# lslrh/DynaMask

Measured on AMD Instinct MI355X. Metric: img/s (DynaMask mask-head path, 512 RoIs/img, fixed 28x28 exit; ms_per_step = ms per RoI batch), higher is better.
Workload: dtype f32

## Files before the change

dynamask_amd/csrc/deform_conv.hip:

```cpp
#include "common.h"

namespace {

struct DcnArgs {
  const float* x;
  const float* offset;
  int NB, C, H, W, HW, Q;
  const float* wp;
  int Cout, CoutP, KQ, dg, relu;
  int q_begin = 0;
  float* out;
  int MT;
  float* ws = nullptr;
  long long ws_stride = 0, ws_floats = 0;
  int ksplit = 1, kchan = 0;
  const float* w2t = nullptr;
  const float* b2 = nullptr;
  float* out2 = nullptr;
  int M2 = 0, w2_ld = 0, out2_ct = 0, store_out = 1;
};

__device__ __forceinline__ float dcn_bilinear(float wt0, float wt1, float wb0, float wb1, float ta, float tb, float ba, float bb) {
  return __builtin_fmaf(wb1, bb, __builtin_fmaf(wb0, ba, __builtin_fmaf(wt1, tb, wt0 * ta)));
}

template <int WGM, int WGN, int WM, int WN>
__global__ __launch_bounds__(WGM* WGN * 64) void deform_conv_kernel(DcnArgs a) {
  constexpr int CK = 8;
  constexpr int TM = WGM * WM * 32;
  constexpr int TN = WGN * WN * 32;
  constexpr int NT = WGM * WGN * 64;
  constexpr int TG = NT / TN;
  constexpr int MAXT = (9 + TG - 1) / TG;
  constexpr int A_F4 = 9 * 2 * TM;
  constexpr int A_PER_T = (A_F4 + NT - 1) / NT;
  static_assert(NT % TN == 0, "threads must tile the pixel columns");

  extern __shared__ __attribute__((aligned(16))) float lds[];
  const int kc_begin = (a.ksplit > 1) ? (int)blockIdx.y * a.kchan : 0;
  const int kc_end = (a.ksplit > 1) ? min(a.C, kc_begin + a.kchan) : a.C;
  float* const e_out = (a.ksplit > 1) ? a.ws + (size_t)blockIdx.y * a.ws_stride : a.out;
  const int e_relu = (a.ksplit > 1) ? 0 : a.relu;
  dm_f32x4* ldsA = reinterpret_cast<dm_f32x4*>(lds);
  dm_f32x4* ldsB = reinterpret_cast<dm_f32x4*>(lds) + A_F4;

  const int tid = threadIdx.x;
  const int lane = tid & 63, wave = tid >> 6;
  const int wave_m = wave / WGN, wave_n = wave % WGN;
  const int hi = lane >> 5, l31 = lane & 31;
  int m_tile, n_tile;
  {
    const int b = blockIdx.x, grp = 8 * a.MT;
    const int full = (gridDim.x / grp) * grp;
    if (b < full) {
      const int g = b / grp, r = b - g * grp;
      m_tile = r / 8;
      n_tile = g * 8 + (r & 7);
    } else {
      const int r = b - full;
      m_tile = r % a.MT;
      n_tile = full / a.MT + r / a.MT;
    }
  }
  const int m0 = m_tile * TM;
  const int q0 = a.q_begin + n_tile * TN;
  const int HW = a.HW, W = a.W, H = a.H;

  int col_n[WN], col_p[WN];
  bool col_ok[WN];
#pragma unroll
  for (int wn = 0; wn < WN; ++wn) {
    int q = q0 + (wave_n * WN + wn) * 32 + l31;
    col_ok[wn] = q < a.Q;
    q = min(q, a.Q - 1);
    col_n[wn] = q / HW;
    col_p[wn] = q - col_n[wn] * HW;
  }

  const int gj = tid % TN;
  const int tg = tid / TN;
  int gq = q0 + gj;
  const bool g_ok = gq < a.Q;
  gq = min(gq, a.Q - 1);
  const int gn = gq / HW;
  const int gp = gq - gn * HW;
  const int gy = gp / W, gx = gp - gy * W;

  int ot[MAXT], ob[MAXT];
  float wt0[MAXT], wt1[MAXT], wb0[MAXT], wb1[MAXT];
  int cur_group = -1;
  const int cpg = a.C / a.dg;

  auto load_params = [&](int group) {
    const float* offp = a.offset + ((size_t)gn * a.dg + group) * 18 * HW + gp;
#pragma unroll
    for (int t = 0; t < MAXT; ++t) {
      const int tap = tg + t * TG;
      ot[t] = ob[t] = 0;
      wt0[t] = wt1[t] = wb0[t] = wb1[t] = 0.f;
      if (tap < 9 && g_ok) {
        const int ki = tap / 3, kj = tap - ki * 3;
        const float off_h = offp[(size_t)(2 * tap) * HW];
        const float off_w = offp[(size_t)(2 * tap + 1) * HW];
        const float h_im = (float)(gy - 1 + ki) + off_h;
        const float w_im = (float)(gx - 1 + kj) + off_w;
        if (h_im > -1.f && w_im > -1.f && h_im < (float)H && w_im < (float)W) {
          const int h_low = (int)floorf(h_im), w_low = (int)floorf(w_im);
          const float lh = h_im - (float)h_low, lw = w_im - (float)w_low;
          const float hh = 1.f - lh, hw = 1.f - lw;
          const float wr_t = (h_low >= 0) ? hh : 0.f;
          const float wr_b = (h_low + 1 <= H - 1) ? lh : 0.f;
          const int rt = min(max(h_low, 0), H - 1), rbm = min(max(h_low + 1, 0), H - 1);
          const int cb = min(max(w_low, 0), W - 2);
          const float wc0 = (cb == w_low ? hw : 0.f) + (cb == w_low + 1 ? lw : 0.f);
          const float wc1 = (cb + 1 == w_low ? hw : 0.f) + (cb + 1 == w_low + 1 ? lw : 0.f);
          ot[t] = rt * W + cb;
          ob[t] = rbm * W + cb;
          wt0[t] = wr_t * wc0; wt1[t] = wr_t * wc1;
          wb0[t] = wr_b * wc0; wb1[t] = wr_b * wc1;
        }
      }
    }
  };

  dm_f32x16 acc[WM][WN];
#pragma unroll
  for (int i = 0; i < WM; ++i)
#pragma unroll
    for (int j = 0; j < WN; ++j)
#pragma unroll
      for (int r = 0; r < 16; ++r) acc[i][j][r] = 0.f;

  struct __attribute__((packed, aligned(4))) F2 { float a, b; };
  dm_f32x4 ra[A_PER_T];
  dm_f32x4 raw[MAXT * 4];
  dm_f32x4 rb0[MAXT];

  auto prefetch_a = [&](int c0) {
#pragma unroll
    for (int i = 0; i < A_PER_T; ++i) {
      const int idx = tid + i * NT;
      dm_f32x4 v = {0.f, 0.f, 0.f, 0.f};
      if (idx < A_F4) {
        const int m = idx % TM;
        const int tq = idx / TM;
        const int qd = tq & 1;
        const int tap = tq >> 1;
        if (m0 + m < a.CoutP)
          v = *reinterpret_cast<const dm_f32x4*>(a.wp + (((size_t)tap * a.KQ + (c0 >> 2) + qd) * a.CoutP + m0 + m) * 4);
      }
      ra[i] = v;
    }
  };
  auto issue_quad = [&](int c0, int qd) {
    const float* xp = a.x + ((size_t)gn * a.C + c0 + qd * 4) * HW;
#pragma unroll
    for (int t = 0; t < MAXT; ++t) {
#pragma unroll
      for (int e = 0; e < 4; ++e) {
        const float* xc = xp + (size_t)e * HW;
        const F2 top = *reinterpret_cast<const F2*>(xc + ot[t]);
        const F2 bot = *reinterpret_cast<const F2*>(xc + ob[t]);
        dm_f32x4 v = {top.a, top.b, bot.a, bot.b};
        raw[t * 4 + e] = v;
      }
    }
  };
  auto combine = [&](int t) {
    dm_f32x4 v;
#pragma unroll
    for (int e = 0; e < 4; ++e) {
      const dm_f32x4 l = raw[t * 4 + e];
      v[e] = dcn_bilinear(wt0[t], wt1[t], wb0[t], wb1[t], l[0], l[1], l[2], l[3]);
    }
    return v;
  };
  auto commit = [&]() {
#pragma unroll
    for (int i = 0; i < A_PER_T; ++i) {
      const int idx = tid + i * NT;
      if (idx < A_F4) ldsA[idx] = ra[i];
    }
#pragma unroll
    for (int t = 0; t < MAXT; ++t) {
      const int tap = tg + t * TG;
      if (tap < 9) {
        ldsB[(0 * 9 + tap) * TN + gj] = rb0[t];
        ldsB[(1 * 9 + tap) * TN + gj] = combine(t);
      }
    }
  };
  auto load_frag = [&](int tap, dm_f32x4* av, dm_f32x4* bv) {
#pragma unroll
    for (int i = 0; i < WM; ++i) av[i] = ldsA[(tap * 2 + hi) * TM + (wave_m * WM + i) * 32 + l31];
#pragma unroll
    for (int j = 0; j < WN; ++j) bv[j] = ldsB[(hi * 9 + tap) * TN + (wave_n * WN + j) * 32 + l31];
  };
  auto mfma_taps = [&](int t0, int t1) {
    dm_f32x4 av[2][WM], bv[2][WN];
    load_frag(t0, av[0], bv[0]);
#pragma unroll
    for (int tap = t0; tap < t1; ++tap) {
      const int cur = (tap - t0) & 1;
      if (tap + 1 < t1) load_frag(tap + 1, av[cur ^ 1], bv[cur ^ 1]);
#pragma unroll
      for (int e = 0; e < 4; ++e)
#pragma unroll
        for (int i = 0; i < WM; ++i)
#pragma unroll
          for (int j = 0; j < WN; ++j)
            acc[i][j] = __builtin_amdgcn_mfma_f32_32x32x2f32(av[cur][i][e], bv[cur][j][e], acc[i][j], 0, 0, 0);
    }
  };

  cur_group = kc_begin / cpg;
  load_params(cur_group);
  prefetch_a(kc_begin);
  issue_quad(kc_begin, 0);
#pragma unroll
  for (int t = 0; t < MAXT; ++t) rb0[t] = combine(t);
  issue_quad(kc_begin, 1);

  for (int c0 = kc_begin; c0 < kc_end; c0 += CK) {
    commit();
    __syncthreads();
    const int cn = c0 + CK;
    const bool more = cn < kc_end;
    if (more) {
      const int group = cn / cpg;
      if (group != cur_group) {
        cur_group = group;
        load_params(group);
      }
      prefetch_a(cn);
      issue_quad(cn, 0);
    }
    __builtin_amdgcn_sched_barrier(0);
    mfma_taps(0, 4);
    __builtin_amdgcn_sched_barrier(0);
    if (more) {
#pragma unroll
      for (int t = 0; t < MAXT; ++t) rb0[t] = combine(t);
      issue_quad(cn, 1);
    }
    __builtin_amdgcn_sched_barrier(0);
    mfma_taps(4, 9);
    __syncthreads();
  }

  {
    float* pj[WN];
#pragma unroll
    for (int j = 0; j < WN; ++j) pj[j] = e_out + (size_t)col_n[j] * a.Cout * HW + col_p[j];
    const int co_lane = m0 + wave_m * WM * 32 + 4 * hi;
    const size_t off_lane = (size_t)co_lane * HW;
    const bool relu = e_relu != 0;
#pragma unroll
    for (int i = 0; i < WM; ++i) {
#pragma unroll
      for (int r = 0; r < 16; ++r) {
        const int k = i * 32 + (r & 3) + 8 * (r >> 2);
        if (co_lane + k < a.Cout) {
          const size_t o = off_lane + (size_t)k * HW;
#pragma unroll
          for (int j = 0; j < WN; ++j) {
            if (col_ok[j]) {
              float v = acc[i][j][r];
              if (relu) v = fmaxf(v, 0.f);
              pj[j][o] = v;
            }
          }
        }
      }
    }
  }
}

__global__ __launch_bounds__(256, 2) void deform_conv_lds_kernel(DcnArgs a) {
  constexpr int TM = 128, TN = 128, NT = 256;
  constexpr int AS_F4 = 3 * 2 * TM;
  constexpr int BS_F4 = 3 * 2 * TN;
  constexpr int A_PER_T = AS_F4 / NT;
  constexpr int X_PER_T = 4;
  extern __shared__ __attribute__((aligned(16))) float lds[];
  const int kc_begin = (a.ksplit > 1) ? (int)blockIdx.y * a.kchan : 0;
  const int kc_end = (a.ksplit > 1) ? min(a.C, kc_begin + a.kchan) : a.C;
  float* const e_out = (a.ksplit > 1) ? a.ws + (size_t)blockIdx.y * a.ws_stride : a.out;
  const int e_relu = (a.ksplit > 1) ? 0 : a.relu;
  dm_f32x4* ldsA = reinterpret_cast<dm_f32x4*>(lds);
  dm_f32x4* ldsB = ldsA + 2 * AS_F4;
  dm_f32x4* ldsX = ldsB + 2 * BS_F4;

  const int tid = threadIdx.x, lane = tid & 63, wave = tid >> 6;
  const int wave_m = wave >> 1, wave_n = wave & 1;
  const int hi = lane >> 5, l31 = lane & 31;
  int m_tile, n_tile;
  {
    const int b = blockIdx.x, grp = 8 * a.MT;
    const int full = (gridDim.x / grp) * grp;
    if (b < full) {
      const int g = b / grp, r = b - g * grp;
      m_tile = r / 8;
      n_tile = g * 8 + (r & 7);
    } else {
      const int r = b - full;
      m_tile = r % a.MT;
      n_tile = full / a.MT + r / a.MT;
    }
  }
  const int m0 = m_tile * TM, q0 = a.q_begin + n_tile * TN;
  const int HW = a.HW, W = a.W, H = a.H;
  const int n0 = q0 / HW;
  const int xbuf = 2 * 2 * HW;

  int col_n[2], col_p[2];
  bool col_ok[2];
#pragma unroll
  for (int wn = 0; wn < 2; ++wn) {
    int q = q0 + (wave_n * 2 + wn) * 32 + l31;
    col_ok[wn] = q < a.Q;
    q = min(q, a.Q - 1);
    col_n[wn] = q / HW;
    col_p[wn] = q - col_n[wn] * HW;
  }

  const int gj = tid & 127, gh = tid >> 7;
  int gq = q0 + gj;
  const bool g_ok = gq < a.Q;
  gq = min(gq, a.Q - 1);
  const int gn = gq / HW, gp = gq - gn * HW;
  const int gy = gp / W, gx = gp - gy * W;
  const int xbase = ((gn - n0) * 2 + gh) * HW;

  int otb[9];
  float wt0[9], wt1[9], wb0[9], wb1[9];
  const int cpg = a.C / a.dg;
  auto load_params = [&](int group) {
    const float* offp = a.offset + ((size_t)gn * a.dg + group) * 18 * HW + gp;
#pragma unroll
    for (int tap = 0; tap < 9; ++tap) {
      otb[tap] = 0;
      wt0[tap] = wt1[tap] = wb0[tap] = wb1[tap] = 0.f;
      if (g_ok) {
        const int ki = tap / 3, kj = tap - ki * 3;
        const float h_im = (float)(gy - 1 + ki) + offp[(size_t)(2 * tap) * HW];
        const float w_im = (float)(gx - 1 + kj) + offp[(size_t)(2 * tap + 1) * HW];
        if (h_im > -1.f && w_im > -1.f && h_im < (float)H && w_im < (float)W) {
          const int h_low = (int)floorf(h_im), w_low = (int)floorf(w_im);
          const float lh = h_im - (float)h_low, lw = w_im - (float)w_low;
          const float hh = 1.f - lh, hw = 1.f - lw;
          const float wr_t = (h_low >= 0) ? hh : 0.f;
          const float wr_b = (h_low + 1 <= H - 1) ? lh : 0.f;
          const int rt = min(max(h_low, 0), H - 1), rbm = min(max(h_low + 1, 0), H - 1);
          const int cb = min(max(w_low, 0), W - 2);
          const float wc0 = (cb == w_low ? hw : 0.f) + (cb == w_low + 1 ? lw : 0.f);
          const float wc1 = (cb + 1 == w_low ? hw : 0.f) + (cb + 1 == w_low + 1 ? lw : 0.f);
          otb[tap] = (rt * W + cb) | ((rbm * W + cb) << 16);
          wt0[tap] = wr_t * wc0; wt1[tap] = wr_t * wc1;
          wb0[tap] = wr_b * wc0; wb1[tap] = wr_b * wc1;
        }
      }
    }
  };

  dm_f32x16 acc[2][2];
#pragma unroll
  for (int i = 0; i < 2; ++i)
#pragma unroll
    for (int j = 0; j < 2; ++j)
#pragma unroll
      for (int r = 0; r < 16; ++r) acc[i][j][r] = 0.f;

  dm_f32x4 ra[A_PER_T], rx[X_PER_T];
  int x_off[X_PER_T];
#pragma unroll
  for (int i = 0; i < X_PER_T; ++i) {
    const int idx = tid + i * NT;
    const int img = idx / (2 * HW), r = idx - img * 2 * HW;
    const int quad = r / HW, px = r - quad * HW;
    const int ii = (idx < 4 * HW) ? img : 0, qq = (idx < 4 * HW) ? quad : 0, pp = (idx < 4 * HW) ? px : 0;
    x_off[i] = ((min(n0 + ii, a.NB - 1) - n0) * a.C + qq * 4) * HW + pp;
  }
  auto load_a = [&](int c0, int g) {
#pragma unroll
    for (int i = 0; i < A_PER_T; ++i) {
      const int idx = tid + i * NT;
      const int m = idx % TM, tq = idx / TM;
      const int mm = min(m0 + m, a.CoutP - 1);
      ra[i] = *reinterpret_cast<const dm_f32x4*>(a.wp + (((size_t)(3 * g + (tq >> 1)) * a.KQ + (c0 >> 2) + (tq & 1)) * a.CoutP + mm) * 4);
    }
  };
  auto store_a = [&](int slot) {
#pragma unroll
    for (int i = 0; i < A_PER_T; ++i) ldsA[slot * AS_F4 + tid + i * NT] = ra[i];
  };
  auto load_x = [&](int c0) {
    const float* xc = a.x + ((size_t)n0 * a.C + c0) * HW;
#pragma unroll
    for (int i = 0; i < X_PER_T; ++i) {
#pragma unroll
      for (int e = 0; e < 4; ++e) rx[i][e] = xc[x_off[i] + e * HW];
    }
  };
  auto store_x = [&](int buf) {
#pragma unroll
    for (int i = 0; i < X_PER_T; ++i) {
      const int idx = tid + i * NT;
      if (idx < 4 * HW) ldsX[buf * xbuf + idx] = rx[i];
    }
  };
  auto gather3 = [&](int t0, int slot, int buf) {
    const dm_f32x4* xq = ldsX + buf * xbuf + xbase;
#pragma unroll
    for (int u = 0; u < 3; ++u) {
      const int tap = t0 + u;
      const dm_f32x4* pt = xq + (otb[tap] & 0xffff);
      const dm_f32x4* pb = xq + (otb[tap] >> 16);
      const dm_f32x4 tl = pt[0], tr = pt[1], bl = pb[0], br = pb[1];
      dm_f32x4 v;
#pragma unroll
      for (int e = 0; e < 4; ++e) v[e] = dcn_bilinear(wt0[tap], wt1[tap], wb0[tap], wb1[tap], tl[e], tr[e], bl[e], br[e]);
      ldsB[slot * BS_F4 + (u * 2 + gh) * TN + gj] = v;
    }
  };
  auto step = [&](int slot, bool fill, int t0, int gbuf) {
    const dm_f32x4* xq = ldsX + gbuf * xbuf + xbase;
#pragma unroll
    for (int u = 0; u < 3; ++u) {
      dm_f32x4 av[2], bv[2];
#pragma unroll
      for (int i = 0; i < 2; ++i) av[i] = ldsA[slot * AS_F4 + (u * 2 + hi) * TM + (wave_m * 2 + i) * 32 + l31];
#pragma unroll
      for (int j = 0; j < 2; ++j) bv[j] = ldsB[slot * BS_F4 + (u * 2 + hi) * TN + (wave_n * 2 + j) * 32 + l31];
      const int tap = t0 + u;
      dm_f32x4 tl, tr, bl, br;
      if (fill) {
        const dm_f32x4* pt = xq + (otb[tap] & 0xffff);
        const dm_f32x4* pb = xq + (otb[tap] >> 16);
        tl = pt[0]; tr = pt[1]; bl = pb[0]; br = pb[1];
      }
      __builtin_amdgcn_sched_barrier(0);
#pragma unroll
      for (int e = 0; e < 2; ++e)
#pragma unroll
        for (int i = 0; i < 2; ++i)
#pragma unroll
          for (int j = 0; j < 2; ++j) acc[i][j] = __builtin_amdgcn_mfma_f32_32x32x2f32(av[i][e], bv[j][e], acc[i][j], 0, 0, 0);
      __builtin_amdgcn_sched_barrier(0);
      if (fill) {
        dm_f32x4 v;
#pragma unroll
        for (int e = 0; e < 4; ++e) v[e] = dcn_bilinear(wt0[tap], wt1[tap], wb0[tap], wb1[tap], tl[e], tr[e], bl[e], br[e]);
        ldsB[(slot ^ 1) * BS_F4 + (u * 2 + gh) * TN + gj] = v;
      }
      __builtin_amdgcn_sched_barrier(0);
#pragma unroll
      for (int e = 2; e < 4; ++e)
#pragma unroll
        for (int i = 0; i < 2; ++i)
#pragma unroll
          for (int j = 0; j < 2; ++j) acc[i][j] = __builtin_amdgcn_mfma_f32_32x32x2f32(av[i][e], bv[j][e], acc[i][j], 0, 0, 0);
      __builtin_amdgcn_sched_barrier(0);
    }
  };

  int cur_group = kc_begin / cpg;
  load_params(cur_group);
  load_x(kc_begin);
  load_a(kc_begin, 0);
  store_x(0);
  store_a(0);
  load_a(kc_begin, 1);
  __syncthreads();
  gather3(0, 0, 0);
  __syncthreads();
  int slot = 0;
  for (int c0 = kc_begin, buf = 0; c0 < kc_end; c0 += 8, buf ^= 1) {
    const int cn = c0 + 8;
    const bool more = cn < kc_end;
    if (more) load_x(cn);
    store_a(slot ^ 1);
    load_a(c0, 2);
    step(slot, true, 3, buf);
    __syncthreads();
    slot ^= 1;
    store_a(slot ^ 1);
    if (more) {
      load_a(cn, 0);
      store_x(buf ^ 1);
    }
    step(slot, true, 6, buf);
    __syncthreads();
    slot ^= 1;
    if (more) {
      const int group = cn / cpg;
      if (group != cur_group) {
        cur_group = group;
        load_params(group);
      }
      store_a(slot ^ 1);
      load_a(cn, 1);
    }
    step(slot, more, 0, buf ^ 1);
    __syncthreads();
    slot ^= 1;
  }

  {
    float* pj[2];
#pragma unroll
    for (int j = 0; j < 2; ++j) pj[j] = e_out + (size_t)col_n[j] * a.Cout * HW + col_p[j];
    const int co_lane = m0 + wave_m * 64 + 4 * hi;
    const size_t off_lane = (size_t)co_lane * HW;
    const bool relu = e_relu != 0;
#pragma unroll
    for (int i = 0; i < 2; ++i)
#pragma unroll
      for (int r = 0; r < 16; ++r) {
        const int k = i * 32 + (r & 3) + 8 * (r >> 2);
        if (co_lane + k < a.Cout) {
          const size_t o = off_lane + (size_t)k * HW;
#pragma unroll
          for (int j = 0; j < 2; ++j)
            if (col_ok[j]) {
              float v = acc[i][j][r];
              if (relu) v = fmaxf(v, 0.f);
              pj[j][o] = v;
            }
        }
      }
  }
}

constexpr int DCN_NEAR_ROWS = 5;

template <int WM, int WGM, int XR>
__global__ __launch_bounds__(256, 2) void deform_conv_band_kernel(DcnArgs a, int tiles_per_img, int BR) {
  constexpr int TM = WM * WGM * 32, TN = (4 / WGM) * 32, NT = 256;
  constexpr int A_F4 = 9 * 2 * TM;
  constexpr int A_PER_T = (A_F4 + NT - 1) / NT;
  extern __shared__ __attribute__((aligned(16))) float lds[];
  const int kc_begin = (a.ksplit > 1) ? (int)blockIdx.y * a.kchan : 0;
  const int kc_end = (a.ksplit > 1) ? min(a.C, kc_begin + a.kchan) : a.C;
  float* const e_out = (a.ksplit > 1) ? a.ws + (size_t)blockIdx.y * a.ws_stride : a.out;
  const int e_relu = (a.ksplit > 1) ? 0 : a.relu;
  dm_f32x4* ldsA = reinterpret_cast<dm_f32x4*>(lds);
  dm_f32x4* ldsX = reinterpret_cast<dm_f32x4*>(lds) + A_F4;
  const int tid = threadIdx.x, lane = tid & 63, wave = tid >> 6;
  const int hi = lane >> 5, l31 = lane & 31;
  const int wave_m = wave % WGM, wave_n = wave / WGM;
  const int HW = a.HW, W = a.W, H = a.H;
  const int PS = BR * W, PS4 = PS >> 2;
  const int n = blockIdx.x / tiles_per_img, tile = blockIdx.x - n * tiles_per_img;
  const int p0 = tile * TN;
  const int p_end = min(p0 + TN, HW);
  const int y_first = p0 / W, y_last = (p_end - 1) / W;
  const int band_y0 = min(max(y_first - (BR - (y_last - y_first + 1)) / 2, 0), H - BR);
  int gp = p0 + wave_n * 32 + l31;
  const bool g_ok = gp < HW;
  gp = min(gp, HW - 1);
  const int gy = gp / W, gx = gp - gy * W;

  int otb[9];
  float wt0[9], wt1[9], wb0[9], wb1[9];
  unsigned oob = 0, any_oob = 0;
  const int cpg = a.C / a.dg;
  auto load_params = [&](int group) {
    const float* offp = a.offset + ((size_t)n * a.dg + group) * 18 * HW + gp;
    oob = 0;
#pragma unroll
    for (int tap = 0; tap < 9; ++tap) {
      otb[tap] = 0;
      wt0[tap] = wt1[tap] = wb0[tap] = wb1[tap] = 0.f;
      if (g_ok) {
        const int ki = tap / 3, kj = tap - ki * 3;
        const float h_im = (float)(gy - 1 + ki) + offp[(size_t)(2 * tap) * HW];
        const float w_im = (float)(gx - 1 + kj) + offp[(size_t)(2 * tap + 1) * HW];
        if (h_im > -1.f && w_im > -1.f && h_im < (float)H && w_im < (float)W) {
          const int h_low = (int)floorf(h_im), w_low = (int)floorf(w_im);
          const float lh = h_im - (float)h_low, lw = w_im - (float)w_low;
          const float hh = 1.f - lh, hw = 1.f - lw;
          const float wr_t = (h_low >= 0) ? hh : 0.f;
          const float wr_b = (h_low + 1 <= H - 1) ? lh : 0.f;
          const int rt = min(max(h_low, 0), H - 1), rbm = min(max(h_low + 1, 0), H - 1);
          const int cb = min(max(w_low, 0), W - 2);
          const float wc0 = (cb == w_low ? hw : 0.f) + (cb == w_low + 1 ? lw : 0.f);
          const float wc1 = (cb + 1 == w_low ? hw : 0.f) + (cb + 1 == w_low + 1 ? lw : 0.f);
          if (rt >= gy - DCN_NEAR_ROWS && rbm <= gy + DCN_NEAR_ROWS) {
            otb[tap] = ((rt - band_y0) * W + cb) | (((rbm - band_y0) * W + cb) << 16);
            wt0[tap] = wr_t * wc0; wt1[tap] = wr_t * wc1;
            wb0[tap] = wr_b * wc0; wb1[tap] = wr_b * wc1;
          } else {
            oob |= 1u << tap;
          }
        }
      }
    }
    any_oob = 0;
#pragma unroll
    for (int tap = 0; tap < 9; ++tap)
      if (__ballot((oob >> tap) & 1u) != 0ull) any_oob |= 1u << tap;
  };

  dm_f32x16 acc[WM];
#pragma unroll
  for (int i = 0; i < WM; ++i)
#pragma unroll
    for (int r = 0; r < 16; ++r) acc[i][r] = 0.f;

  dm_f32x4 ra[A_PER_T], rx[XR];
  unsigned a_off[A_PER_T];
#pragma unroll
  for (int i = 0; i < A_PER_T; ++i) {
    const int idx = min(tid + i * NT, A_F4 - 1);
    const int m = idx % TM, tq = idx / TM;
    a_off[i] = (unsigned)((((size_t)(tq >> 1) * a.KQ + (tq & 1)) * a.CoutP + min(m, a.CoutP - 1)) * 4);
  }
  auto load_a = [&](int c0) {
    const float* wb = a.wp + (size_t)(c0 >> 2) * a.CoutP * 4;
#pragma unroll
    for (int i = 0; i < A_PER_T; ++i) ra[i] = *reinterpret_cast<const dm_f32x4*>(wb + a_off[i]);
  };
  auto load_x = [&](int c0) {
    const float* xb = a.x + ((size_t)n * a.C + c0) * HW + (size_t)band_y0 * W;
#pragma unroll
    for (int i = 0; i < XR; ++i) {
      const int idx = tid + i * NT;
      const int off = (idx < PS) ? idx : (idx < 2 * PS ? 4 * HW + idx - PS : 0);
#pragma unroll
      for (int e = 0; e < 4; ++e) rx[i][e] = xb[off + e * HW];
    }
  };
  auto store_ax = [&]() {
#pragma unroll
    for (int i = 0; i < A_PER_T; ++i) {
      const int idx = tid + i * NT;
      if (idx < A_F4) ldsA[idx] = ra[i];
    }
#pragma unroll
    for (int i = 0; i < XR; ++i) {
      const int idx = tid + i * NT;
      if (idx < 2 * PS) ldsX[idx] = rx[i];
    }
  };
  struct __attribute__((packed, aligned(4))) F2 { float a, b; };

  int cur_group = kc_begin / cpg;
  load_params(cur_group);
  load_a(kc_begin);
  load_x(kc_begin);
  for (int c0 = kc_begin; c0 < kc_end; c0 += 8) {
    __syncthreads();
    store_ax();
    __syncthreads();
    const int cn = c0 + 8;
    if (cn < kc_end) {
      load_a(cn);
      load_x(cn);
    }
    const unsigned any_oob_s = __builtin_amdgcn_readfirstlane(any_oob);
    const dm_f32x4* pq = ldsX + hi * PS;
    const float* gl = a.x + ((size_t)n * a.C + c0 + 4 * hi) * HW;
    constexpr int AB = (WM < 4) ? 2 : 1;
    dm_f32x4 av[AB][WM];
    dm_f32x4 tl, tr, bl, br;
    auto issue_x = [&](int tap) {
      const dm_f32x4* pt = pq + (otb[tap] & 0xffff);
      const dm_f32x4* pb = pq + (otb[tap] >> 16);
      tl = pt[0]; tr = pt[1]; bl = pb[0]; br = pb[1];
    };
    auto issue_a = [&](int tap) {
#pragma unroll
      for (int i = 0; i < WM; ++i) av[tap % AB][i] = ldsA[(tap * 2 + hi) * TM + (wave_m * WM + i) * 32 + l31];
    };
    issue_x(0);
    issue_a(0);
#pragma unroll
    for (int tap = 0; tap < 9; ++tap) {
      float v[4];
#pragma unroll
      for (int e = 0; e < 4; ++e) v[e] = dcn_bilinear(wt0[tap], wt1[tap], wb0[tap], wb1[tap], tl[e], tr[e], bl[e], br[e]);
      __builtin_amdgcn_sched_barrier(0);
      if (tap + 1 < 9) {
        issue_x(tap + 1);
        if (AB == 2) issue_a(tap + 1);
      }
      __builtin_amdgcn_sched_barrier(0);
#pragma unroll
      for (int e = 0; e < 4; ++e)
#pragma unroll
        for (int i = 0; i < WM; ++i) acc[i] = __builtin_amdgcn_mfma_f32_32x32x2f32(av[tap % AB][i][e], v[e], acc[i], 0, 0, 0);
      __builtin_amdgcn_sched_barrier(0);
      if (AB == 1 && tap + 1 < 9) issue_a(tap + 1);
    }
    if (any_oob_s) {
      const float* offp = a.offset + ((size_t)n * a.dg + cur_group) * 18 * HW + gp;
#pragma unroll 1
      for (int tap = 0; tap < 9; ++tap) {
        if (!((any_oob_s >> tap) & 1u)) continue;
        const bool mine = (oob >> tap) & 1u;
        float w00 = 0.f, w01 = 0.f, w10 = 0.f, w11 = 0.f;
        int g_t = 0, g_b = 0;
        if (mine) {
          const int ki = tap / 3, kj = tap - ki * 3;
          const float h_im = (float)(gy - 1 + ki) + offp[(size_t)(2 * tap) * HW];
          const float w_im = (float)(gx - 1 + kj) + offp[(size_t)(2 * tap + 1) * HW];
          const int h_low = (int)floorf(h_im), w_low = (int)floorf(w_im);
          const float lh = h_im - (float)h_low, lw = w_im - (float)w_low;
          const float hh = 1.f - lh, hw = 1.f - lw;
          const float wr_t = (h_low >= 0) ? hh : 0.f;
          const float wr_b = (h_low + 1 <= H - 1) ? lh : 0.f;
          const int rt = min(max(h_low, 0), H - 1), rbm = min(max(h_low + 1, 0), H - 1);
          const int cb = min(max(w_low, 0), W - 2);
          const float wc0 = (cb == w_low ? hw : 0.f) + (cb == w_low + 1 ? lw : 0.f);
          const float wc1 = (cb + 1 == w_low ? hw : 0.f) + (cb + 1 == w_low + 1 ? lw : 0.f);
          g_t = rt * W + cb;
          g_b = rbm * W + cb;
          w00 = wr_t * wc0; w01 = wr_t * wc1;
          w10 = wr_b * wc0; w11 = wr_b * wc1;
        }
        dm_f32x4 av[WM];
#pragma unroll
        for (int i = 0; i < WM; ++i) av[i] = ldsA[(tap * 2 + hi) * TM + (wave_m * WM + i) * 32 + l31];
#pragma unroll
        for (int e = 0; e < 4; ++e) {
          const float* gc = gl + (size_t)e * HW;
          const F2 top = *reinterpret_cast<const F2*>(gc + g_t);
          const F2 bot = *reinterpret_cast<const F2*>(gc + g_b);
          const float g = dcn_bilinear(w00, w01, w10, w11, top.a, top.b, bot.a, bot.b);
#pragma unroll
          for (int i = 0; i < WM; ++i) acc[i] = __builtin_amdgcn_mfma_f32_32x32x2f32(av[i][e], g, acc[i], 0, 0, 0);
        }
      }
    }
    if (cn < kc_end) {
      const int group = cn / cpg;
      if (group != cur_group) {
        cur_group = group;
        load_params(group);
      }
    }
  }
  if (WGM == 1 && a.w2t) {
    constexpr int MT2 = (WM + 1) / 2;
    const int ld2 = a.w2_ld;
    __syncthreads();
    {
      const dm_f32x4* src = reinterpret_cast<const dm_f32x4*>(a.w2t);
      dm_f32x4* dst = reinterpret_cast<dm_f32x4*>(lds);
      for (int idx = tid; idx < a.Cout * (ld2 / 4); idx += NT) dst[idx] = src[idx];
    }
    __syncthreads();
    const float* w2t = lds;
    dm_f32x16 acc2[MT2];
#pragma unroll
    for (int t = 0; t < MT2; ++t)
#pragma unroll
      for (int r = 0; r < 16; ++r) acc2[t][r] = 0.f;
#pragma unroll
    for (int i = 0; i < WM; ++i)
#pragma unroll
      for (int r = 0; r < 16; ++r) {
        const int kb = i * 32 + (r & 3) + 8 * (r >> 2) + 4 * hi;
        const float b = fmaxf(acc[i][r], 0.f);
#pragma unroll
        for (int t = 0; t < MT2; ++t)
          if (t * 32 < ld2) acc2[t] = __builtin_amdgcn_mfma_f32_32x32x2f32(w2t[kb * ld2 + t * 32 + l31], b, acc2[t], 0, 0, 0);
      }
    const int p = p0 + wave_n * 32 + l31;
    if (p < HW) {
      float* po2 = a.out2 + (size_t)n * a.out2_ct * HW + p;
#pragma unroll
      for (int t = 0; t < MT2; ++t)
#pragma unroll
        for (int r = 0; r < 16; ++r) {
          const int co = t * 32 + (r & 3) + 8 * (r >> 2) + 4 * hi;
          if (co < a.M2) po2[(size_t)co * HW] = fmaxf(acc2[t][r] + a.b2[co], 0.f);
        }
    }
    if (!a.store_out) return;
  }
  {
    const int p = p0 + wave_n * 32 + l31;
    if (p < HW) {
      float* po = e_out + (size_t)n * a.Cout * HW + p;
      const bool relu = e_relu != 0;
#pragma unroll
      for (int i = 0; i < WM; ++i)
#pragma unroll
        for (int r = 0; r < 16; ++r) {
          const int co = (wave_m * WM + i) * 32 + (r & 3) + 8 * (r >> 2) + 4 * hi;
          if (co < a.Cout) {
            float v = acc[i][r];
            if (relu) v = fmaxf(v, 0.f);
            po[(size_t)co * HW] = v;
          }
        }
    }
  }
}

__global__ __launch_bounds__(256) void dcn_splitk_reduce_kernel(const float* __restrict__ ws, int splits, long long stride,
                                                               long long total, int relu, float* __restrict__ out) {
  const bool v4 = splits > 0;
  splits = v4 ? splits : -splits;
  if (v4) {
    const float4* ws4 = reinterpret_cast<const float4*>(ws);
    float4* out4 = reinterpret_cast<float4*>(out);
    const long long total4 = total >> 2, stride4 = stride >> 2;
    for (long long e = (long long)blockIdx.x * blockDim.x + threadIdx.x; e < total4; e += (long long)gridDim.x * blockDim.x) {
      float4 v = ws4[e];
      for (int s_ = 1; s_ < splits; ++s_) {
        const float4 w = ws4[(size_t)s_ * stride4 + e];
        v.x += w.x; v.y += w.y; v.z += w.z; v.w += w.w;
      }
      if (relu) { v.x = fmaxf(v.x, 0.f); v.y = fmaxf(v.y, 0.f); v.z = fmaxf(v.z, 0.f); v.w = fmaxf(v.w, 0.f); }
      out4[e] = v;
    }
    return;
  }
  for (long long e = (long long)blockIdx.x * blockDim.x + threadIdx.x; e < total; e += (long long)gridDim.x * blockDim.x) {
    float v = ws[e];
    for (int s_ = 1; s_ < splits; ++s_) v += ws[(size_t)s_ * stride + e];
    out[e] = relu ? fmaxf(v, 0.f) : v;
  }
}

static void dcn_choose_split(DcnArgs& a, long long wgs, long long slots, long long ws_floats, bool lds_tiles = false) {
  a.ksplit = 1;
  if (!a.ws || a.q_begin != 0 || wgs <= 0) return;
  const int chunks = a.C / 8;
  const long long per = (long long)a.NB * a.Cout * a.HW;
  int S = 1;
  if (a.NB <= 24) {
    long long Smax = min(min(8LL, slots / wgs), (long long)chunks / 2);
    if (per > 0) Smax = min(Smax, ws_floats / per);
    const double chain_us = chunks * 3.5, out_mb = (double)per * 4e-6;
    double best = 8.0;
    for (int c = 2; c <= Smax; ++c) {
      const double g = chain_us * (1.0 - 1.0 / c) - (5.0 + (c + 1) * out_mb * 0.25);
      if (g > best) { best = g; S = c; }
    }
  } else if (lds_tiles && wgs < slots && chunks >= 12 && per > 0 && ws_floats / per >= 3) {
    S = 3;
  }
  if (S >= 2) {
    const int per_split = dm_ceil_div(chunks, S);
    a.kchan = per_split * 8;
    a.ksplit = dm_ceil_div(chunks, per_split);
    a.ws_stride = per;
  }
}

static int dcn_finish_split(const DcnArgs& a, int relu, float* out, hipStream_t st) {
  if (a.ksplit <= 1) return dm_check_launch();
  int rc = dm_check_launch();
  if (rc != DM_OK) return rc;
  const long long total = a.ws_stride;
  const bool v4 = (total & 3) == 0 && ((((uintptr_t)a.ws) | ((uintptr_t)out)) & 15) == 0;
  DM_LAUNCH(dcn_splitk_reduce_kernel, dim3((unsigned)min((long long)4096, ((v4 ? total / 4 : total) + 255) / 256)), dim3(256), 0, st, a.ws,
            v4 ? a.ksplit : -a.ksplit, a.ws_stride, total, relu, out);
  return dm_check_launch();
}

template <int WM, int WGM, int XR>
int launch_dcn_band(DcnArgs& a, hipStream_t st) {
  const int BR = 16;
  if (8 * BR * a.W / 4 > XR * 256 || a.H < BR) return DM_ERR_UNSUPPORTED;
  const int tiles = dm_ceil_div(a.HW, (4 / WGM) * 32);
  const size_t lds_bytes = 16 * (size_t)(9 * 2 * WM * WGM * 32) + 4 * (size_t)8 * BR * a.W;
  if (a.w2t) {
    if (WGM != 1 || a.w2_ld != dm_ceil_div(a.M2, 32) * 32 || a.w2_ld > (WM + 1) / 2 * 32 || (size_t)a.Cout * a.w2_ld * 4 > lds_bytes ||
        a.Cout != WM * 32)
      return DM_ERR_UNSUPPORTED;
    a.ws = nullptr;
  }
  dcn_choose_split(a, (long long)a.NB * tiles, 2LL * dm_num_cus(), a.ws_floats);
  DM_LAUNCH((deform_conv_band_kernel<WM, WGM, XR>), dim3((unsigned)(a.NB * tiles), (unsigned)a.ksplit), dim3(256), lds_bytes, st, a, tiles, BR);
  return dcn_finish_split(a, a.relu, a.out, st);
}

template <int WGM, int WGN, int WM, int WN>
int launch_dcn(DcnArgs& a, hipStream_t st) {
  constexpr int TM = WGM * WM * 32;
  constexpr int TN = WGN * WN * 32;
  constexpr int NT = WGM * WGN * 64;
  a.MT = dm_ceil_div(a.CoutP, TM);
  const int NTiles = dm_ceil_div(a.Q - a.q_begin, TN);
  const size_t lds_bytes = 16 * ((size_t)9 * 2 * TM + (size_t)2 * 9 * TN);
  static bool attr_set[DM_MAX_DEVICES] = {false};
  if (lds_bytes > 64 * 1024 &&
      dm_ensure_lds_limit(reinterpret_cast<const void*>(&deform_conv_kernel<WGM, WGN, WM, WN>), (int)lds_bytes, attr_set) != DM_OK)
    return DM_ERR_LAUNCH;
  dcn_choose_split(a, (long long)a.MT * NTiles, (NT == 256 ? 2LL : 1LL) * dm_num_cus(), a.ws_floats);
  DM_LAUNCH((deform_conv_kernel<WGM, WGN, WM, WN>), dim3(a.MT * NTiles, a.ksplit), dim3(NT), lds_bytes, st, a);
  return dcn_finish_split(a, a.relu, a.out, st);
}

}

struct DcnTout {
  const float* w2t = nullptr;
  const float* b2 = nullptr;
  float* out2 = nullptr;
  int M2 = 0, out2_ct = 0;
};
static int deform_conv_fwd_impl(const float* x, const float* offset, int NB, int C, int H, int W,
                                const float* w_packed, int Cout, int deform_groups, int relu, float* out, float* ws,
                                long long ws_floats, dm_stream_t stream, const DcnTout* tout = nullptr);

extern "C" int dm_deform_conv_fwd(const float* x, const float* offset, int NB, int C, int H, int W,
                                  const float* w_packed, int Cout, int deform_groups, int relu, float* out,
                                  dm_stream_t stream) {
  return deform_conv_fwd_impl(x, offset, NB, C, H, W, w_packed, Cout, deform_groups, relu, out, nullptr, 0, stream);
}

extern "C" long long dm_deform_conv_splitk_floats(int NB, int C, int H, int W, int Cout) {
  if (NB <= 0 || C < 32 || H <= 0 || W <= 0 || Cout <= 0) return 0;
  const long long wgs = (long long)dm_ceil_div(Cout, 128) * dm_ceil_div((long long)NB * H * W, 128);
  if (wgs * 2 > 2LL * dm_num_cus() && !(H * W <= 256 && wgs < 2LL * dm_num_cus())) return 0;
  return 8LL * NB * Cout * H * W;
}

extern "C" int dm_deform_conv_fwd_ws(const float* x, const float* offset, int NB, int C, int H, int W,
                                     const float* w_packed, int Cout, int deform_groups, int relu, float* out,
                                     float* workspace, long long workspace_floats, dm_stream_t stream) {
  return deform_conv_fwd_impl(x, offset, NB, C, H, W, w_packed, Cout, deform_groups, relu, out, workspace, workspace_floats, stream);
}

static bool dcn_tout_shape_ok(int NB, int C, int H, int W, int Cout, int M2) {
  if (NB <= 0 || C <= 0 || H <= 0 || W <= 0 || Cout != C || M2 <= 0) return false;
  const int HW = H * W, CoutP = dm_conv_packed_cout(Cout);
  const int max_rows = (W - 1 + 128 + W - 1) / W;
  if (!(H >= 16 && (W & 3) == 0 && 8 * 16 * W / 4 <= 7 * 256 && (16 - max_rows) / 2 >= DCN_NEAR_ROWS && HW > 256 && HW < 65536 &&
        (CoutP == 64 || CoutP == 128) && Cout > 32 && Cout == CoutP))
    return false;
  const bool narrow = 8 * 16 * W / 4 <= 4 * 256;
  const bool few = (long long)NB * dm_ceil_div(HW, 128) * 4 < (long long)dm_num_cus() * 3;
  if (few) return false;
  if (CoutP == 128 && !narrow) return false;
  return dm_ceil_div(M2, 32) <= (CoutP / 32 + 1) / 2;
}

extern "C" int dm_deform_conv_tout_supported(int NB, int C, int H, int W, int Cout, int M2) {
  return dcn_tout_shape_ok(NB, C, H, W, Cout, M2) ? 1 : 0;
}

extern "C" int dm_deform_conv_tout_fwd(const float* x, const float* offset, int NB, int C, int H, int W, const float* w_packed,
                                       int Cout, int deform_groups, const float* w2t, const float* b2, int M2, float* out2,
                                       int out2_ch_total, float* out_dcn, dm_stream_t stream) {
  if (!w2t || !b2 || !out2 || M2 <= 0 || M2 > out2_ch_total) return DM_ERR_INVALID_ARG;
  if (NB == 0) return DM_OK;
  if (!dcn_tout_shape_ok(NB, C, H, W, Cout, M2)) return DM_ERR_UNSUPPORTED;
  DcnTout t;
  t.w2t = w2t; t.b2 = b2; t.out2 = out2; t.M2 = M2; t.out2_ct = out2_ch_total;
  return deform_conv_fwd_impl(x, offset, NB, C, H, W, w_packed, Cout, deform_groups, 1, out_dcn ? out_dcn : out2, nullptr, 0, stream,
                              &t) ;
}

static int deform_conv_fwd_impl(const float* x, const float* offset, int NB, int C, int H, int W,
                                const float* w_packed, int Cout, int deform_groups, int relu, float* out, float* ws,
                                long long ws_floats, dm_stream_t stream, const DcnTout* tout) {
  if (!x || !offset || !w_packed || !out) return DM_ERR_INVALID_ARG;
  if (relu & 16) return DM_ERR_UNSUPPORTED;
  if (NB < 0 || C <= 0 || H <= 0 || W <= 0 || Cout <= 0 || deform_groups <= 0 || C % deform_groups != 0)
    return DM_ERR_INVALID_ARG;
  if ((long long)NB * H * W > 0x7fffffffLL) return DM_ERR_INVALID_ARG;
  if ((C / deform_groups) % 8 != 0) return DM_ERR_UNSUPPORTED;
  if (W < 2) return DM_ERR_UNSUPPORTED;
  if (NB == 0) return DM_OK;
  DcnArgs a;
  a.x = x; a.offset = offset; a.NB = NB; a.C = C; a.H = H; a.W = W; a.HW = H * W; a.Q = NB * H * W;
  a.wp = w_packed; a.Cout = Cout; a.CoutP = dm_conv_packed_cout(Cout); a.KQ = (C + 7) / 8 * 2; a.dg = deform_groups;
  a.relu = relu & 1; a.out = out;
  a.ws = (ws && ws_floats > 0) ? ws : nullptr;
  a.ws_floats = a.ws ? ws_floats : 0;
  if (tout) {
    a.w2t = tout->w2t; a.b2 = tout->b2; a.out2 = tout->out2; a.M2 = tout->M2; a.w2_ld = dm_ceil_div(tout->M2, 32) * 32;
    a.out2_ct = tout->out2_ct;
    a.store_out = (out != tout->out2) ? 1 : 0;
  }
  hipStream_t st = (hipStream_t)stream;
  {
    const int max_rows = (W - 1 + 128 + W - 1) / W;
    if (H >= 16 && (W & 3) == 0 && 8 * 16 * W / 4 <= 7 * 256 && (16 - max_rows) / 2 >= DCN_NEAR_ROWS && a.HW > 256 &&
        a.HW < 65536 && (a.CoutP == 64 || a.CoutP == 128) && Cout > 32) {
      const bool narrow = 8 * 16 * W / 4 <= 4 * 256;
      bool few = (long long)NB * dm_ceil_div(a.HW, 128) * 4 < (long long)dm_num_cus() * 3;
      if (few && a.ws && NB <= 24 && !tout) few = false;
      if (a.CoutP == 64) {
        if (few) return narrow ? launch_dcn_band<1, 2, 4>(a, st) : launch_dcn_band<1, 2, 7>(a, st);
        return narrow ? launch_dcn_band<2, 1, 4>(a, st) : launch_dcn_band<2, 1, 7>(a, st);
      }
      if (few) return narrow ? launch_dcn_band<1, 4, 4>(a, st) : launch_dcn_band<1, 4, 7>(a, st);
      return narrow ? launch_dcn_band<4, 1, 4>(a, st) : launch_dcn_band<2, 2, 7>(a, st);
    }
  }
  if (tout) return DM_ERR_UNSUPPORTED;
  const bool lds_split = a.ws && Cout > 64 && a.HW >= 128 && a.HW <= 256 && (a.HW & 3) == 0;
  if (!lds_split && Cout > 64 &&
      (long long)dm_ceil_div(a.CoutP, 128) * dm_ceil_div(a.Q, 128) * 20 <= (long long)dm_num_cus() * 9)
    return launch_dcn<2, 2, 1, 1>(a, st);
  if (Cout > 64 && a.HW >= 128 && a.HW <= 256 && (a.HW & 3) == 0 && (C / deform_groups) % 8 == 0) {
    a.MT = dm_ceil_div(a.CoutP, 128);
    const int NTiles = dm_ceil_div(a.Q, 128);
    const size_t lds_bytes = 16 * ((size_t)2 * 2 * 3 * 2 * 128) + (size_t)4 * 2 * 2 * 8 * a.HW;
    static bool attr_lds[DM_MAX_DEVICES] = {false};
    if (dm_ensure_lds_limit(reinterpret_cast<const void*>(&deform_conv_lds_kernel), 16 * 2 * 2 * 3 * 2 * 128 + 4 * 2 * 2 * 8 * 256,
                            attr_lds) != DM_OK)
      return DM_ERR_LAUNCH;
    static const int tail_mode = getenv("DM_DCN_TAIL") ? atoi(getenv("DM_DCN_TAIL")) : 1;
    const int slots = 2 * dm_num_cus();
    const int full_rounds = (a.MT * NTiles) / slots;
    const int rem = a.MT * NTiles - full_rounds * slots;
    if (tail_mode && !(relu & 8) && full_rounds >= 1 && rem > 0 && rem * 20 <= 3 * slots) {
      const int n_main = full_rounds * slots / a.MT;
      const int Q = a.Q;
      a.Q = n_main * 128;
      DM_LAUNCH(deform_conv_lds_kernel, dim3(a.MT * n_main), dim3(256), lds_bytes, st, a);
      int rc = dm_check_launch();
      if (rc != DM_OK) return rc;
      a.q_begin = a.Q;
      a.Q = Q;
      return launch_dcn<2, 2, 1, 1>(a, st);
    }
    dcn_choose_split(a, (long long)a.MT * NTiles, slots, a.ws_floats, true);
    DM_LAUNCH(deform_conv_lds_kernel, dim3(a.MT * NTiles, a.ksplit), dim3(256), lds_bytes, st, a);
    return dcn_finish_split(a, a.relu, a.out, st);
  }
  if (Cout > 64 && (long long)dm_ceil_div(a.CoutP, 128) * dm_ceil_div(a.Q, 64) * 20 <= (long long)dm_num_cus() * 9)
    return launch_dcn<2, 2, 1, 1>(a, st);
  if (Cout > 64) return launch_dcn<2, 2, 2, 1>(a, st);
  if (Cout > 32) return launch_dcn<2, 2, 1, 1>(a, st);
  return launch_dcn<1, 4, 1, 1>(a, st);
}
```

Before: 279.1.

## Add Cout=256 deform-conv kernel sharing one bilinear sample tile across all channels

```diff
diff --git a/dynamask_amd/csrc/deform_conv.hip b/dynamask_amd/csrc/deform_conv.hip
--- a/dynamask_amd/csrc/deform_conv.hip
+++ b/dynamask_amd/csrc/deform_conv.hip
@@ -19,6 +19,8 @@
   float* out2 = nullptr;
   int M2 = 0, w2_ld = 0, out2_ct = 0, store_out = 1;
 };
+
+typedef float dm_f32x2 __attribute__((ext_vector_type(2)));
 
 __device__ __forceinline__ float dcn_bilinear(float wt0, float wt1, float wb0, float wb1, float ta, float tb, float ba, float bb) {
   return __builtin_fmaf(wb1, bb, __builtin_fmaf(wb0, ba, __builtin_fmaf(wt1, tb, wt0 * ta)));
@@ -513,6 +515,237 @@
     const int co_lane = m0 + wave_m * 64 + 4 * hi;
     const size_t off_lane = (size_t)co_lane * HW;
     const bool relu = e_relu != 0;
+#pragma unroll
+    for (int i = 0; i < 2; ++i)
+#pragma unroll
+      for (int r = 0; r < 16; ++r) {
+        const int k = i * 32 + (r & 3) + 8 * (r >> 2);
+        if (co_lane + k < a.Cout) {
+          const size_t o = off_lane + (size_t)k * HW;
+#pragma unroll
+          for (int j = 0; j < 2; ++j)
+            if (col_ok[j]) {
+              float v = acc[i][j][r];
+              if (relu) v = fmaxf(v, 0.f);
+              pj[j][o] = v;
+            }
+        }
+      }
+  }
+}
+
+__global__ __launch_bounds__(256, 2) void deform_conv_c256_kernel(DcnArgs a) {
+  constexpr int TN = 64, NT = 256;
+  constexpr int BS_F4 = 3 * 2 * TN;
+  constexpr int X_PER_T = 4;
+  extern __shared__ __attribute__((aligned(16))) float lds[];
+  dm_f32x4* ldsB = reinterpret_cast<dm_f32x4*>(lds);
+  dm_f32x4* ldsX = ldsB + 2 * BS_F4;
+
+  const int tid = threadIdx.x, lane = tid & 63, wave = tid >> 6;
+  const int hi = lane >> 5, l31 = lane & 31;
+  const int q0 = a.q_begin + (int)blockIdx.x * TN;
+  const int HW = a.HW, W = a.W, H = a.H;
+  const int n0 = q0 / HW;
+  const int xbuf = 2 * 2 * HW;
+
+  const int gj = tid & 63, gh = (tid >> 6) & 1, rb = tid >> 7;
+  int gq = q0 + gj;
+  const bool g_ok = gq < a.Q;
+  gq = min(gq, a.Q - 1);
+  const int gn = gq / HW, gp = gq - gn * HW;
+  const int gy = gp / W, gx = gp - gy * W;
+  const int xbase = ((gn - n0) * 2 + gh) * HW;
+
+  int otb[3][2];
+  float wt0[3][2], wt1[3][2], wb0[3][2], wb1[3][2];
+  const int cpg = a.C / a.dg;
+  auto load_params = [&](int group) {
+    const float* offp = a.offset + ((size_t)gn * a.dg + group) * 18 * HW + gp;
+#pragma unroll
+    for (int s = 0; s < 3; ++s)
+#pragma unroll
+      for (int r = 0; r < 2; ++r) {
+        otb[s][r] = 0;
+        wt0[s][r] = wt1[s][r] = wb0[s][r] = wb1[s][r] = 0.f;
+        if (g_ok) {
+          const int ki = s, kj = r ? 2 : rb, tap = 3 * s + kj;
+          const float h_im = (float)(gy - 1 + ki) + offp[(size_t)(2 * tap) * HW];
+          const float w_im = (float)(gx - 1 + kj) + offp[(size_t)(2 * tap + 1) * HW];
+          if (h_im > -1.f && w_im > -1.f && h_im < (float)H && w_im < (float)W) {
+            const int h_low = (int)floorf(h_im), w_low = (int)floorf(w_im);
+            const float lh = h_im - (float)h_low, lw = w_im - (float)w_low;
+            const float hh = 1.f - lh, hw = 1.f - lw;
+            const float wr_t = (h_low >= 0) ? hh : 0.f;
+            const float wr_b = (h_low + 1 <= H - 1) ? lh : 0.f;
+            const int rt = min(max(h_low, 0), H - 1), rbm = min(max(h_low + 1, 0), H - 1);
+            const int cb = min(max(w_low, 0), W - 2);
+            const float wc0 = (cb == w_low ? hw : 0.f) + (cb == w_low + 1 ? lw : 0.f);
+            const float wc1 = (cb + 1 == w_low ? hw : 0.f) + (cb + 1 == w_low + 1 ? lw : 0.f);
+            otb[s][r] = (rt * W + cb) | ((rbm * W + cb) << 16);
+            wt0[s][r] = wr_t * wc0; wt1[s][r] = wr_t * wc1;
+            wb0[s][r] = wr_b * wc0; wb1[s][r] = wr_b * wc1;
+          }
+        }
+      }
+  };
+
+  dm_f32x16 acc[2][2];
+#pragma unroll
+  for (int i = 0; i < 2; ++i)
+#pragma unroll
+    for (int j = 0; j < 2; ++j)
+#pragma unroll
+      for (int r = 0; r < 16; ++r) acc[i][j][r] = 0.f;
+
+  dm_f32x4 rx[X_PER_T];
+  const __amdgpu_buffer_rsrc_t xsrc = __builtin_amdgcn_make_buffer_rsrc(
+      const_cast<float*>(a.x) + (size_t)n0 * a.C * HW, 0, min(2, a.NB - n0) * a.C * HW * 4, 0x00020000);
+  const __amdgpu_buffer_rsrc_t wsrc = __builtin_amdgcn_make_buffer_rsrc(const_cast<float*>(a.wp), 0, 9 * a.KQ * a.CoutP * 16, 0x00020000);
+  unsigned x_off[X_PER_T];
+#pragma unroll
+  for (int i = 0; i < X_PER_T; ++i) {
+    const int idx = tid + i * NT;
+    const int img = idx / (2 * HW), r = idx - img * 2 * HW;
+    const int quad = r / HW, px = r - quad * HW;
+    const int ii = (idx < 4 * HW) ? img : 0, qq = (idx < 4 * HW) ? quad : 0, pp = (idx < 4 * HW) ? px : 0;
+    x_off[i] = 4u * (unsigned)(((min(n0 + ii, a.NB - 1) - n0) * a.C + qq * 4) * HW + pp);
+  }
+  unsigned a_off[2];
+#pragma unroll
+  for (int i = 0; i < 2; ++i) a_off[i] = 16u * (unsigned)(hi * a.CoutP + min(wave * 64 + i * 32 + l31, a.CoutP - 1));
+  const int a_quad = a.CoutP * 16, a_tap = a.KQ * a_quad;
+  auto load_a1 = [&](dm_f32x4 (&dst)[6], int c0, int g, int u) {
+    const int so = (3 * g + u) * a_tap + (c0 >> 2) * a_quad;
+#pragma unroll
+    for (int i = 0; i < 2; ++i) dst[u * 2 + i] = __builtin_bit_cast(dm_f32x4, __builtin_amdgcn_raw_buffer_load_b128(wsrc, a_off[i], so, 0));
+  };
+  auto load_x = [&](int c0) {
+#pragma unroll
+    for (int e = 0; e < 4; ++e) {
+      const int so = (c0 + e) * HW * 4;
+#pragma unroll
+      for (int i = 0; i < X_PER_T; ++i) rx[i][e] = __builtin_bit_cast(float, __builtin_amdgcn_raw_buffer_load_b32(xsrc, x_off[i], so, 0));
+    }
+  };
+  auto store_x = [&](int buf) {
+#pragma unroll
+    for (int i = 0; i < X_PER_T; ++i) {
+      const int idx = tid + i * NT;
+      if (idx < 4 * HW) ldsX[buf * xbuf + idx] = rx[i];
+    }
+  };
+  auto whole_read = [&](const dm_f32x4* xq, int s, dm_f32x4& tl, dm_f32x4& tr, dm_f32x4& bl, dm_f32x4& br) {
+    const dm_f32x4* pt = xq + (otb[s][0] & 0xffff);
+    const dm_f32x4* pb = xq + (otb[s][0] >> 16);
+    tl = pt[0]; tr = pt[1]; bl = pb[0]; br = pb[1];
+  };
+  auto whole_write = [&](int slot, int s, const dm_f32x4& tl, const dm_f32x4& tr, const dm_f32x4& bl, const dm_f32x4& br) {
+    dm_f32x4 v;
+#pragma unroll
+    for (int e = 0; e < 4; ++e) v[e] = dcn_bilinear(wt0[s][0], wt1[s][0], wb0[s][0], wb1[s][0], tl[e], tr[e], bl[e], br[e]);
+    ldsB[slot * BS_F4 + (rb * 2 + gh) * TN + gj] = v;
+  };
+  auto half_read = [&](const dm_f32x4* xq, int s, dm_f32x2& tl, dm_f32x2& tr, dm_f32x2& bl, dm_f32x2& br) {
+    const dm_f32x2* pt = reinterpret_cast<const dm_f32x2*>(xq + (otb[s][1] & 0xffff)) + rb;
+    const dm_f32x2* pb = reinterpret_cast<const dm_f32x2*>(xq + (otb[s][1] >> 16)) + rb;
+    tl = pt[0]; tr = pt[2]; bl = pb[0]; br = pb[2];
+  };
+  auto half_write = [&](int slot, int s, const dm_f32x2& tl, const dm_f32x2& tr, const dm_f32x2& bl, const dm_f32x2& br) {
+    dm_f32x2 v;
+#pragma unroll
+    for (int e = 0; e < 2; ++e) v[e] = dcn_bilinear(wt0[s][1], wt1[s][1], wb0[s][1], wb1[s][1], tl[e], tr[e], bl[e], br[e]);
+    reinterpret_cast<dm_f32x2*>(&ldsB[slot * BS_F4 + (2 * 2 + gh) * TN + gj])[rb] = v;
+  };
+  auto step = [&](const dm_f32x4 (&cur)[6], dm_f32x4 (&nxt)[6], int slot, bool fill, int sn, int gbuf, bool pre, int pc0, int pg) {
+    const dm_f32x4* xq = ldsX + gbuf * xbuf + xbase;
+#pragma unroll
+    for (int u = 0; u < 3; ++u) {
+      dm_f32x4 bv[2];
+#pragma unroll
+      for (int j = 0; j < 2; ++j) bv[j] = ldsB[slot * BS_F4 + (u * 2 + hi) * TN + j * 32 + l31];
+      dm_f32x4 tl, tr, bl, br;
+      dm_f32x2 htl, htr, hbl, hbr;
+      if (fill && u == 0) whole_read(xq, sn, tl, tr, bl, br);
+      if (fill && u == 1) half_read(xq, sn, htl, htr, hbl, hbr);
+      if (pre) load_a1(nxt, pc0, pg, u);
+      __builtin_amdgcn_sched_barrier(0);
+#pragma unroll
+      for (int e = 0; e < 2; ++e)
+#pragma unroll
+        for (int i = 0; i < 2; ++i)
+#pragma unroll
+          for (int j = 0; j < 2; ++j) acc[i][j] = __builtin_amdgcn_mfma_f32_32x32x2f32(cur[u * 2 + i][e], bv[j][e], acc[i][j], 0, 0, 0);
+      __builtin_amdgcn_sched_barrier(0);
+      if (fill && u == 0) whole_write(slot ^ 1, sn, tl, tr, bl, br);
+      if (fill && u == 1) half_write(slot ^ 1, sn, htl, htr, hbl, hbr);
+      __builtin_amdgcn_sched_barrier(0);
+#pragma unroll
+      for (int e = 2; e < 4; ++e)
+#pragma unroll
+        for (int i = 0; i < 2; ++i)
+#pragma unroll
+          for (int j = 0; j < 2; ++j) acc[i][j] = __builtin_amdgcn_mfma_f32_32x32x2f32(cur[u * 2 + i][e], bv[j][e], acc[i][j], 0, 0, 0);
+      __builtin_amdgcn_sched_barrier(0);
+    }
+  };
+  int cur_group = 0;
+  auto chunk = [&](dm_f32x4 (&p)[6], dm_f32x4 (&q)[6], int c0, int buf, int slot) {
+    const int cn = c0 + 8;
+    const bool more = cn < a.C;
+    if (more) load_x(cn);
+    step(p, q, slot, true, 1, buf, true, c0, 1);
+    __syncthreads();
+    if (more) store_x(buf ^ 1);
+    step(q, p, slot ^ 1, true, 2, buf, true, c0, 2);
+    __syncthreads();
+    if (more) {
+      const int group = cn / cpg;
+      if (group != cur_group) {
+        cur_group = group;
+        load_params(group);
+      }
+    }
+    step(p, q, slot, more, 0, buf ^ 1, more, cn, 0);
+    __syncthreads();
+  };
+
+  dm_f32x4 a0[6], a1[6];
+  load_params(0);
+  load_x(0);
+#pragma unroll
+  for (int u = 0; u < 3; ++u) load_a1(a0, 0, 0, u);
+  store_x(0);
+  __syncthreads();
+  {
+    const dm_f32x4* xq = ldsX + xbase;
+    dm_f32x4 tl, tr, bl, br;
+    dm_f32x2 htl, htr, hbl, hbr;
+    whole_read(xq, 0, tl, tr, bl, br);
+    half_read(xq, 0, htl, htr, hbl, hbr);
+    whole_write(0, 0, tl, tr, bl, br);
+    half_write(0, 0, htl, htr, hbl, hbr);
+  }
+  __syncthreads();
+  for (int c0 = 0; c0 < a.C; c0 += 16) {
+    chunk(a0, a1, c0, 0, 0);
+    if (c0 + 8 < a.C) chunk(a1, a0, c0 + 8, 1, 1);
+  }
+
+  {
+    float* pj[2];
+    bool col_ok[2];
+#pragma unroll
+    for (int j = 0; j < 2; ++j) {
+      int q = q0 + j * 32 + l31;
+      col_ok[j] = q < a.Q;
+      q = min(q, a.Q - 1);
+      const int n = q / HW;
+      pj[j] = a.out + (size_t)n * a.Cout * HW + (q - n * HW);
+    }
+    const int co_lane = wave * 64 + 4 * hi;
+    const size_t off_lane = (size_t)co_lane * HW;
+    const bool relu = a.relu != 0;
 #pragma unroll
     for (int i = 0; i < 2; ++i)
 #pragma unroll
@@ -897,6 +1130,28 @@
   return dcn_finish_split(a, a.relu, a.out, st);
 }
 
+int launch_dcn_c256(DcnArgs& a, bool tail, hipStream_t st) {
+  const size_t lds_bytes = 16 * ((size_t)2 * 3 * 2 * 64) + (size_t)4 * 2 * 2 * 8 * a.HW;
+  const int NTiles = dm_ceil_div(a.Q, 64);
+  const int slots = 2 * dm_num_cus();
+  const int full_rounds = NTiles / slots;
+  const int rem = NTiles - full_rounds * slots;
+  a.ksplit = 1;
+  if (tail && full_rounds >= 1 && rem > 0 && rem * 20 <= 3 * slots) {
+    const int n_main = full_rounds * slots;
+    const int Q = a.Q;
+    a.Q = n_main * 64;
+    DM_LAUNCH(deform_conv_c256_kernel, dim3(n_main), dim3(256), lds_bytes, st, a);
+    int rc = dm_check_launch();
+    if (rc != DM_OK) return rc;
+    a.q_begin = a.Q;
+    a.Q = Q;
+    return launch_dcn<2, 2, 1, 1>(a, st);
+  }
+  DM_LAUNCH(deform_conv_c256_kernel, dim3(NTiles), dim3(256), lds_bytes, st, a);
+  return dm_check_launch();
+}
+
 }
 
 struct DcnTout {
@@ -1011,6 +1266,10 @@
       return DM_ERR_LAUNCH;
     static const int tail_mode = getenv("DM_DCN_TAIL") ? atoi(getenv("DM_DCN_TAIL")) : 1;
     const int slots = 2 * dm_num_cus();
+    if (a.CoutP == 256) {
+      dcn_choose_split(a, (long long)a.MT * NTiles, slots, a.ws_floats, true);
+      if (a.ksplit == 1) return launch_dcn_c256(a, tail_mode && !(relu & 8), st);
+    }
     const int full_rounds = (a.MT * NTiles) / slots;
     const int rem = a.MT * NTiles - full_rounds * slots;
     if (tail_mode && !(relu & 8) && full_rounds >= 1 && rem > 0 && rem * 20 <= 3 * slots) {
```

Result: faster. 287.2 (median of 6 runs) (+2.9%).
